# xuekt98/BBDM

Hardware: NVIDIA H100
Metric: denoising-steps/sec (UNet fwd) at 256^2 pixel-BBDM (higher is better)
Workload: dtype bf16x3 (split-bf16 tensor-core products, fp32 accumulate: fp32-class)

## Files before the change

bbdm_b200/cabi.py:

```python
from __future__ import annotations

import ctypes as C
import os

import torch

_HERE = os.path.dirname(os.path.abspath(__file__))
LIB_PATH = os.environ.get("BBDM_LIB") or os.path.join(_HERE, "libbbdm_b200.so")

ABI_VERSION = 3
OBJ = {"grad": 0, "noise": 1, "ysubx": 2}
RESAMPLE_NONE, RESAMPLE_UP2, RESAMPLE_DOWN2 = 0, 1, 2
RES_NONE, RES_SAME, RES_UP2, RES_DOWN2 = 0, 1, 2, 3
GN_MAX_SLICES = 64
ATTN_HEAD_DIMS = (16, 32, 64, 128)
ATTN_TC_HEAD_DIMS = (64, 128)
LN_MAX_C = 2048


def layernorm_bwd_workspace(rows, C):
    return -(-rows // 64) * 2 * C

SYMBOLS = [
    "bbdm_abi_version", "bbdm_last_error", "bbdm_device_info", "bbdm_check_device_fault",
    "bbdm_bridge_q_sample", "bbdm_bridge_p_sample", "bbdm_bridge_p_sample_dev", "bbdm_nchw_to_nhwc_cat", "bbdm_nhwc_to_nchw",
    "bbdm_gather_rows", "bbdm_linear_f32", "bbdm_gn_stats", "bbdm_prep_operand",
    "bbdm_pack_weight_split", "bbdm_pack_weight_split_padded", "bbdm_pack_weight_split_taps", "bbdm_pack_weight_split_dgrad",
    "bbdm_pack_weight_f32", "bbdm_conv_umma", "bbdm_conv_direct",
    "bbdm_attention", "bbdm_attention_split", "bbdm_attention_tc", "bbdm_conv_umma_geometry", "bbdm_gn_finalize_partials",
    "bbdm_split_grad", "bbdm_conv_wgrad_workspace", "bbdm_conv_wgrad", "bbdm_gn_bwd_reduce", "bbdm_gn_bwd_apply",
    "bbdm_conv_wgrad_direct", "bbdm_attention_bwd", "bbdm_conv_direct_pad", "bbdm_softmax_rows_split", "bbdm_vq_nearest", "bbdm_s2d_split", "bbdm_pack_weight_split_both",
    "bbdm_wino_geometry", "bbdm_wino_input", "bbdm_wino_output", "bbdm_wino_pack_weight",
    "bbdm_wino6_geometry", "bbdm_wino6_input", "bbdm_wino6_output", "bbdm_wino6_pack_weight",
# ... 20 lines not shown


class ConvArgs(C.Structure):
    _fields_ = [("B", C.c_int), ("H", C.c_int), ("W", C.c_int),
                ("Cin", C.c_int), ("Cout", C.c_int), ("taps", C.c_int),
                ("a_hi", C.c_void_p), ("a_lo", C.c_void_p), ("w_hi", C.c_void_p), ("w_lo", C.c_void_p),
                ("bias", C.c_void_p),
                ("Cin2", C.c_int),
                ("a2_hi", C.c_void_p), ("a2_lo", C.c_void_p), ("w2_hi", C.c_void_p), ("w2_lo", C.c_void_p),
                ("bias2", C.c_void_p),
                ("residual", C.c_void_p), ("res_mode", C.c_int),
                ("out", C.c_void_p), ("out_hi", C.c_void_p), ("out_lo", C.c_void_p),
                ("passes", C.c_int), ("out_nchw_channels", C.c_int), ("upsample2x", C.c_int),
                ("stats_partial", C.c_void_p), ("weights_per_image", C.c_int), ("operand_f16", C.c_int)]


class WinoInputArgs(C.Structure):
    _fields_ = [("src1", C.c_void_p), ("c1", C.c_int), ("src2", C.c_void_p), ("c2", C.c_int),
                ("B", C.c_int), ("H", C.c_int), ("W", C.c_int), ("groups", C.c_int),
                ("mean", C.c_void_p), ("rstd", C.c_void_p), ("gamma", C.c_void_p), ("beta", C.c_void_p),
                ("film_scale", C.c_void_p), ("film_shift", C.c_void_p), ("film_stride", C.c_int64),
                ("silu", C.c_int),
                ("v_hi", C.c_void_p), ("v_lo", C.c_void_p), ("raw_hi", C.c_void_p), ("raw_lo", C.c_void_p),
                ("act_hi", C.c_void_p), ("act_lo", C.c_void_p)]


class WinoOutputArgs(C.Structure):
    _fields_ = [("m", C.c_void_p), ("inv_wscale", C.c_void_p), ("B", C.c_int), ("H", C.c_int), ("W", C.c_int), ("Cout", C.c_int),
                ("bias", C.c_void_p), ("residual", C.c_void_p), ("res_mode", C.c_int),
                ("out", C.c_void_p), ("stats_partial", C.c_void_p), ("up2_phases", C.c_int)]


class BbdmError(RuntimeError):
    pass


_lib = None


def load():
    global _lib
    if _lib is not None:
        return _lib
    if not os.path.exists(LIB_PATH):
        raise BbdmError(
            f"{LIB_PATH} not found: build the sm_90a kernels first (python -m bbdm_b200.build). "
            "bbdm_b200 has no PyTorch/CPU fallback for its kernels.")
# ... 108 lines not shown
    return cls


LAUNCHES = {"n": 0}


def _req(t, dtype=torch.float32):
    assert t.is_cuda and t.is_contiguous() and t.dtype == dtype, (t.device, t.dtype, t.is_contiguous())
    return t


@_guard_all
class CudaBackend:

    name = "sm_90a"
    requires_cuda = True
    wino_tensor_scale = True
    wino_tiles = (4, 6)

    def __init__(self):
        self.lib = load()

    def empty(self, shape, dtype, device):
        return torch.empty(shape, dtype=dtype, device=device)

    def q_sample(self, x0, y, noise, t, m_t, var_t, objective, xt_out, obj_out):
        B = x0.shape[0]
        n = x0.numel() // B
        for z in (x0, y, noise, m_t, var_t, xt_out, obj_out):
            _req(z)
        _req(t, torch.int64)
        check(self.lib.bbdm_bridge_q_sample(ptr(x0), ptr(y), ptr(noise), ptr(t), ptr(m_t), ptr(var_t),
                                            m_t.numel(), OBJ[objective], ptr(xt_out), ptr(obj_out), B, n,
                                            stream()))
        LAUNCHES["n"] += 1

    def p_sample(self, x_t, y, eps, noise, coef, objective, clip, is_last, x_out, x0_out):
        for z in (x_t, y, eps, x_out):
            _req(z)
        c = PSampleCoef(*[float(v) for v in coef])
        check(self.lib.bbdm_bridge_p_sample(ptr(x_t), ptr(y), ptr(eps), ptr(noise), c, OBJ[objective],
                                            int(clip), int(is_last), ptr(x_out), ptr(x0_out), x_t.numel(),
                                            stream()))
        LAUNCHES["n"] += 1

    def p_sample_dev(self, x_t, y, eps, noise, coef_dev, objective, clip, is_last, x_out, x0_out):
        for z in (x_t, y, eps, x_out, coef_dev):
# ... 78 lines not shown
        a = ConvArgs(B, H, W, Cin, Cout, taps, ptr(a_hi), ptr(a_lo), ptr(w_hi), ptr(w_lo), ptr(bias),
                     Cin2, ptr(a2_hi), ptr(a2_lo), ptr(w2_hi), ptr(w2_lo), ptr(bias2),
                     ptr(residual), res_mode, ptr(out), ptr(out_hi), ptr(out_lo), passes, out_nchw_channels,
                     int(upsample2x), ptr(stats_partial), int(weights_per_image), int(operand_f16))
        check(self.lib.bbdm_conv_umma(C.byref(a), stream()))
        LAUNCHES["n"] += 1

    def conv_geometry(self, H, W):
        v = [C.c_int(0) for _ in range(4)]
        check(self.lib.bbdm_conv_umma_geometry(H, W, *[C.byref(z) for z in v]))
        return tuple(z.value for z in v)

    def _wino(self, name, tile):
        assert tile in self.wino_tiles, tile
        return getattr(self.lib, f"bbdm_wino{'' if tile == 4 else tile}_{name}")

    def wino_geometry(self, B, H, W, tile=4):
        th, tw, el, tot = C.c_int(0), C.c_int(0), C.c_int(0), C.c_int64(0)
        check(self._wino("geometry", tile)(B, H, W, C.byref(th), C.byref(tw), C.byref(tot), C.byref(el)))
        return th.value, tw.value, tot.value, bool(el.value)

    def wino_input(self, src1, src2, *, groups=32, mean=None, rstd=None, gamma=None, beta=None, film_scale=None,
                   film_shift=None, film_stride=0, silu=True, v_hi, v_lo, raw_hi=None, raw_lo=None, act_hi=None,
                   act_lo=None, tile=4):
        B, H, W, c1 = src1.shape
        a = WinoInputArgs(ptr(_req(src1)), c1, ptr(src2), 0 if src2 is None else src2.shape[3], B, H, W, groups,
                          ptr(mean), ptr(rstd), ptr(gamma), ptr(beta), ptr(film_scale), ptr(film_shift), film_stride,
                          int(silu), ptr(_req(v_hi, torch.float16)), ptr(_req(v_lo, torch.float16)),
                          ptr(raw_hi), ptr(raw_lo), ptr(act_hi), ptr(act_lo))
        check(self._wino("input", tile)(C.byref(a), stream()))
        LAUNCHES["n"] += 1

    def wino_output(self, m, *, B, H, W, Cout, bias=None, residual=None, res_mode=RES_NONE, out, stats_partial=None,
                    inv_wscale=None, tile=4, up2_phases=False):
        a = WinoOutputArgs(ptr(_req(m)), None if inv_wscale is None else ptr(_req(inv_wscale)), B, H, W, Cout, ptr(bias), ptr(residual), res_mode, ptr(_req(out)),
                           ptr(stats_partial), int(up2_phases))
        check(self._wino("output", tile)(C.byref(a), stream()))
        LAUNCHES["n"] += 1

    def wino_pack_weight(self, w, u_hi, u_lo, dgrad=False, inv_wscale=None, tile=4):
        Cout, Cin = w.shape[0], w.shape[1]
        check(self._wino("pack_weight", tile)(ptr(_req(w)), Cout, Cin, int(dgrad), ptr(_req(u_hi, torch.float16)),
                                              ptr(_req(u_lo, torch.float16)),
                                              None if inv_wscale is None else ptr(_req(inv_wscale)), stream()))
        LAUNCHES["n"] += 1

    def layernorm_split(self, x, gamma, beta, eps, out_f32=None, out_hi=None, out_lo=None):
        Cc = x.shape[-1]
        check(self.lib.bbdm_layernorm_split(ptr(_req(x)), x.numel() // Cc, Cc, ptr(_req(gamma)), ptr(_req(beta)), eps,
                                            ptr(out_f32), ptr(out_hi), ptr(out_lo), stream()))
        LAUNCHES["n"] += 1

# ... 177 lines not shown
```

bbdm_b200/convs.py:

```python
from __future__ import annotations

import os

import torch

from . import cabi
from .weights import upsample_phase_weights

WINOGRAD = os.environ.get("BBDM_WINOGRAD", "1") != "0"
WINOGRAD_TRAIN = os.environ.get("BBDM_WINOGRAD_TRAIN", "1") != "0"
WINO_MIN_C = int(os.environ.get("BBDM_WINO_MIN_C", "256"))
WINO_MIN_TILES = int(os.environ.get("BBDM_WINO_MIN_TILES", "512"))


def wino_channels_ok(cin, cout, min_c):
    return cin % 64 == 0 and cout % 64 == 0 and min(cin, cout) >= min_c


def wino_tile(H, W):
    f6 = 64 * (-(-H // 6)) * (-(-W // 6))
    f4 = 36 * (H / 4) * (W / 4)
    return 6 if f6 <= 0.9 * f4 else 4


def winograd_ok(geometry, cin, cout, min_c, min_tiles, tile=4):
    th, tw, tiles, ok = geometry
    px = tile * tile
    return bool(ok and wino_channels_ok(cin, cout, min_c) and (th * tw * px >= 128 * 16 or tiles * px >= min_tiles * 16))


class FreshBuffers:

    def __init__(self, device):
        self.device = device

    def get(self, shape, dtype=torch.float32):
        return torch.empty(shape, dtype=dtype, device=self.device)

    def put(self, *ts):
        pass


def wino_conv(be, pool, geometry, src1, src2, *, cout, planes=None, weight=None, dgrad=False, bias=None,
              residual=None, res_mode=cabi.RES_NONE, stats=False, tile=4, up2_phases=False, **transform):
    B, H, W, c1 = src1.shape
    cin = c1 + (0 if src2 is None else src2.shape[3])
    th, _, mtot, _ = geometry
    npos = (tile + 2) ** 2
    tkw = {} if tile == 4 else dict(tile=tile)
    assert not up2_phases or (tile == 6 and planes is not None and residual is None)
    ncols = 4 * cout if up2_phases else cout
    v_hi, v_lo = pool.get((npos, mtot, cin), torch.float16), pool.get((npos, mtot, cin), torch.float16)
    be.wino_input(src1, src2, v_hi=v_hi, v_lo=v_lo, **transform, **tkw)
    if planes is None:
        u_hi, u_lo = pool.get((npos, cout, cin), torch.float16), pool.get((npos, cout, cin), torch.float16)
        u_inv = pool.get((1,)) if getattr(be, "wino_tensor_scale", False) else None
        be.wino_pack_weight(weight.detach().contiguous(), u_hi, u_lo, dgrad=dgrad,
                            **({} if u_inv is None else dict(inv_wscale=u_inv)), **tkw)
    else:
        u_hi, u_lo, u_inv = planes
        assert u_hi.shape[0] == npos, (u_hi.shape, tile)
    m = pool.get((npos, mtot, ncols))
    be.conv_umma(B=npos, H=mtot // 16, W=16, Cin=cin, Cout=ncols, taps=1, a_hi=v_hi, a_lo=v_lo, w_hi=u_hi, w_lo=u_lo,
                 out=m, passes=3, weights_per_image=True, operand_f16=True)
    pool.put(v_hi, v_lo)
    f = 2 if up2_phases else 1
    rows = 4 * th if up2_phases else th
    out = pool.get((B, f * H, f * W, cout))
    part = pool.get((B * rows, cout, 2)) if stats else None
    if up2_phases:
        tkw["up2_phases"] = True
    be.wino_output(m, B=B, H=H, W=W, Cout=cout, bias=bias, residual=residual, res_mode=res_mode, out=out,
                   stats_partial=part, **({} if u_inv is None else dict(inv_wscale=u_inv)), **tkw)
# ... 75 lines not shown
```

bbdm_b200/csrc/winograd.cu:

```cuda
#include "common.cuh"
#include <cuda_fp16.h>
#include <stdlib.h>

namespace bbdm {

constexpr float WINO_WSCALE_FIXED = 256.0f;

__host__ __device__ inline float wino_wscale(uint32_t mbits) {
  if (mbits == 0) return WINO_WSCALE_FIXED;
  const int e = (int)(mbits >> 23) - 127;
  int k = 14 - (e + ((mbits & 0x7fffffu) != 0 ? 1 : 0));
  k = k < -100 ? -100 : (k > 100 ? 100 : k);
  float s = 1.0f;
  for (; k > 0; --k) s *= 2.0f;
  for (; k < 0; ++k) s *= 0.5f;
  return s;
}

template <int S>
__device__ __forceinline__ void wino_bt6(float* d) {
  const float d0 = d[0], d1 = d[S], d2 = d[2 * S], d3 = d[3 * S], d4 = d[4 * S], d5 = d[5 * S];
  d[0] = fmaf(4.0f, d0, fmaf(-5.0f, d2, d4));
  d[S] = fmaf(-4.0f, d1 + d2, d3 + d4);
  d[2 * S] = fmaf(4.0f, d1 - d2, d4 - d3);
// ... 32 lines not shown
  const float a = m[S] + m[2 * S], b = m[S] - m[2 * S];
  const float c = m[3 * S] + m[4 * S], d = m[3 * S] - m[4 * S];
  const float e = m[5 * S] + m[6 * S], f = m[5 * S] - m[6 * S];
  y[0] = ((m[0] + a) + c) + e;
  y[T] = fmaf(2.0f, d, fmaf(0.5f, f, b));
  y[2 * T] = fmaf(4.0f, c, fmaf(0.25f, e, a));
  y[3 * T] = fmaf(8.0f, d, fmaf(0.125f, f, b));
  y[4 * T] = fmaf(16.0f, c, fmaf(0.0625f, e, a));
  y[5 * T] = fmaf(32.0f, d, fmaf(0.03125f, f, b)) + m[7 * S];
}

__device__ __forceinline__ void split2_f16(float a, float b, uint32_t& hi, uint32_t& lo) {
  const __half2 h = __floats2half2_rn(a, b);
  const float2 hf = __half22float2(h);
  const __half2 l = __floats2half2_rn(a - hf.x, b - hf.y);
  hi = *reinterpret_cast<const uint32_t*>(&h);
  lo = *reinterpret_cast<const uint32_t*>(&l);
}

struct WinoInParams {
  const float* src1; int c1;
  const float* src2; int c2;
  int B, H, W, C, groups, cpg, th, tw;
  int64_t Mtot;
  const float* mean; const float* rstd; const float* gamma; const float* beta;
  const float* fscale; const float* fshift; int64_t fstride;
  int silu;
  __half* v_hi; __half* v_lo;
  __nv_bfloat16* raw_hi; __nv_bfloat16* raw_lo;
  __nv_bfloat16* act_hi; __nv_bfloat16* act_lo;
  unsigned long long* fault;
};

constexpr unsigned long long WINO6_RANGE_FAULT = 0xC0000000ull;

template <int VEC>
__global__ void __launch_bounds__(256)
wino_input_kernel(const WinoInParams p) {
  const int b = blockIdx.x / p.th, ty = blockIdx.x % p.th;
  const int c = (blockIdx.y * 256 + threadIdx.x) * VEC;
  if (c >= p.C) return;
  float sc[VEC], sh[VEC];
#pragma unroll
  for (int v = 0; v < VEC; ++v) {
    const int g = (c + v) / p.cpg;
    const float s0 = p.rstd[b * p.groups + g] * p.gamma[c + v];
// ... 89 lines not shown
        const __half h = __float2half_rn(t[0][q]);
        p.v_hi[off] = h;
        p.v_lo[off] = __float2half_rn(t[0][q] - __half2float(h));
      }
    }
  }
}

template <int T>
struct WinoIn {
  static constexpr int N = T + 2;
  static constexpr int CC = 64;
  static constexpr int TX = T == 4 ? 8 : 4;
  static constexpr int COLS = T * TX + 2;
  static constexpr int PATCH = N * COLS * CC;
  static constexpr size_t SMEM = 2 * (size_t)PATCH * sizeof(float);
};
static_assert(WinoIn<4>::SMEM == 2 * 6 * 34 * 64 * 4 && WinoIn<6>::SMEM * 2 <= 227 * 1024, "staged patch budget");

__device__ __forceinline__ void cp_async16(uint32_t saddr, const void* g) {
  asm volatile("cp.async.cg.shared.global [%0], [%1], 16;" ::"r"(saddr), "l"(g) : "memory");
}

template <int T>
__global__ void __launch_bounds__(256, 2)
wino_input_smem_kernel(const WinoInParams p) {
  using K = WinoIn<T>;
  constexpr int N = K::N, CC = K::CC, TX = K::TX, COLS = K::COLS;
  extern __shared__ __align__(16) float patch[];
  const int b = blockIdx.x / p.th, ty = blockIdx.x % p.th;
  const int cbase = blockIdx.y * CC;
  const float* base;
  int cs, cc0;
  if (cbase < p.c1) { base = p.src1; cs = p.c1; cc0 = cbase; } else { base = p.src2; cs = p.c2; cc0 = cbase - p.c1; }
  const int y0 = T * ty - 1;
  const int tid = threadIdx.x;
  const int ch4 = tid & 15;
  const int pix0 = tid >> 4;
  constexpr int NPIX = N * COLS;

  if constexpr (T == 6) {
    if (blockIdx.x == 0) {
      const int64_t tiles = (int64_t)p.B * p.th * p.tw;
      const int npad = (int)(p.Mtot - tiles);
      for (int k = tid; k < N * N * npad * CC; k += 256) {
        const int c = k % CC, r = (k / CC) % npad, q = k / (CC * npad);
        const int64_t off = ((int64_t)q * p.Mtot + tiles + r) * p.C + cbase + c;
        p.v_hi[off] = __float2half_rn(0.f);
        p.v_lo[off] = __float2half_rn(0.f);
      }
    }
  }

  float sc[4], sh[4];
#pragma unroll
  for (int v = 0; v < 4; ++v) {
    sc[v] = 1.0f; sh[v] = 0.0f;
    if (p.mean) {
      const int c = cbase + ch4 * 4 + v;
      const int g = c / p.cpg;
      const float s0 = p.rstd[b * p.groups + g] * p.gamma[c];
      const float h0 = p.beta[c] - p.mean[b * p.groups + g] * s0;
      float f1 = 1.0f, f0 = 0.0f;
      if (p.fscale) { f1 = 1.0f + p.fscale[(int64_t)b * p.fstride + c]; f0 = p.fshift[(int64_t)b * p.fstride + c]; }
      sc[v] = s0 * f1;
      sh[v] = fmaf(h0, f1, f0);
    }
  }
  const int nseg = (p.tw + TX - 1) / TX;
  const uint32_t patch_s = (uint32_t)__cvta_generic_to_shared(patch);

  auto stage = [&](int seg, int buf) {
    const int x0 = T * TX * seg - 1;
    int i = 0, j = pix0;
    for (int px = pix0; px < NPIX; px += 16, j += 16) {
      if (j >= COLS) { j -= COLS; ++i; }
      const int iy = y0 + i, ix = x0 + j;
      if (iy >= 0 && iy < p.H && ix >= 0 && ix < p.W)
        cp_async16(patch_s + (uint32_t)(((buf * NPIX + px) * CC + ch4 * 4) * 4),
                   base + (((int64_t)b * p.H + iy) * p.W + ix) * cs + cc0 + ch4 * 4);
    }
    asm volatile("cp.async.commit_group;" ::: "memory");
  };

  stage(0, 0);
  for (int seg = 0; seg < nseg; ++seg) {
    const int buf = seg & 1;
    if (seg + 1 < nseg) {
      stage(seg + 1, buf ^ 1);
      asm volatile("cp.async.wait_group 1;" ::: "memory");
    } else {
      asm volatile("cp.async.wait_group 0;" ::: "memory");
    }
    __syncthreads();
    float* pb = patch + buf * K::PATCH;
    const int x0 = T * TX * seg - 1;
    int i = 0, j = pix0;
    for (int px = pix0; px < NPIX; px += 16, j += 16) {
      if (j >= COLS) { j -= COLS; ++i; }
      const int iy = y0 + i, ix = x0 + j;
      float4* q = reinterpret_cast<float4*>(pb + px * CC + ch4 * 4);
      float4 a = make_float4(0.f, 0.f, 0.f, 0.f);
      if (iy >= 0 && iy < p.H && ix >= 0 && ix < p.W) {
        const float4 x = *q;
        if (p.raw_hi && i >= 1 && i <= T && j >= 1 && j <= T * TX) {
          uint2 h, l;
          split4(x, h, l);
          const int64_t off = (((int64_t)b * p.H + iy) * p.W + ix) * p.C + cbase + ch4 * 4;
          *reinterpret_cast<uint2*>(p.raw_hi + off) = h;
          *reinterpret_cast<uint2*>(p.raw_lo + off) = l;
        }
        a.x = fmaf(x.x, sc[0], sh[0]); a.y = fmaf(x.y, sc[1], sh[1]);
        a.z = fmaf(x.z, sc[2], sh[2]); a.w = fmaf(x.w, sc[3], sh[3]);
        if (p.silu) {
          a.x = __fdividef(a.x, 1.0f + __expf(-a.x)); a.y = __fdividef(a.y, 1.0f + __expf(-a.y));
          a.z = __fdividef(a.z, 1.0f + __expf(-a.z)); a.w = __fdividef(a.w, 1.0f + __expf(-a.w));
        }
        if (p.act_hi && i >= 1 && i <= T && j >= 1 && j <= T * TX) {
          uint2 h, l;
          split4(a, h, l);
          const int64_t off = (((int64_t)b * p.H + iy) * p.W + ix) * p.C + cbase + ch4 * 4;
          *reinterpret_cast<uint2*>(p.act_hi + off) = h;
          *reinterpret_cast<uint2*>(p.act_lo + off) = l;
        }
      }
      *q = a;
    }
    __syncthreads();
    const int64_t plane = p.Mtot * p.C;
    if constexpr (T == 4) {
      const int txl = tid >> 5, c0 = (tid & 31) * 2;
      const int tx = TX * seg + txl;
      if (tx < p.tw) {
        float t0[36], t1[36];
#pragma unroll
        for (int i = 0; i < 6; ++i)
#pragma unroll
          for (int j = 0; j < 6; ++j) {
            const float2 v = *reinterpret_cast<const float2*>(pb + ((i * COLS + 4 * txl + j) * CC + c0));
            t0[i * 6 + j] = v.x;
// ... 315 lines not shown
        u_lo[off] = l;
      }
    }
  }
}

}

using namespace bbdm;

namespace {

template <int T>
int wino_geometry_t(int B, int H, int W, int* tiles_h, int* tiles_w, int64_t* tiles_total, int* eligible) {
  BBDM_REQUIRE(B > 0 && H > 0 && W > 0, "wino_geometry: bad shape");
  const int th = T == 4 ? H / 4 : (H + 5) / 6, tw = T == 4 ? W / 4 : (W + 5) / 6;
  int64_t mtot = (int64_t)B * th * tw;
  if (T == 6) mtot = mtot < 128 ? 128 : (mtot + 15) / 16 * 16;
  if (tiles_h) *tiles_h = th;
  if (tiles_w) *tiles_w = tw;
  if (tiles_total) *tiles_total = mtot;
  const bool aligned = T == 6 || (H % 4 == 0 && W % 4 == 0);
  if (eligible) *eligible = (aligned && mtot % 16 == 0 && mtot >= 128) ? 1 : 0;
  return BBDM_OK;
}

template <int T>
int wino_input_t(const BbdmWinoInputArgs* a, void* stream) {
  BBDM_REQUIRE(a && a->src1 && a->v_hi && a->v_lo, "wino_input: null args");
  WinoInParams p;
  p.src1 = a->src1; p.c1 = a->c1;
  p.src2 = a->src2; p.c2 = a->src2 ? a->c2 : 0;
  p.B = a->B; p.H = a->H; p.W = a->W;
  p.C = p.c1 + p.c2;
  p.groups = a->groups;
  if (T == 4)
    BBDM_REQUIRE(p.B > 0 && p.H > 0 && p.W > 0 && p.H % 4 == 0 && p.W % 4 == 0, "wino_input: H, W must be multiples of 4");
  else
    BBDM_REQUIRE(p.B > 0 && p.H > 0 && p.W > 0, "wino6_input: bad shape");
  BBDM_REQUIRE(p.c1 % 2 == 0 && p.c2 % 2 == 0 && p.C > 0, "wino_input: channel counts must be even");
  if (a->mean) {
    BBDM_REQUIRE(a->rstd && a->gamma && a->beta && p.groups > 0 && p.C % p.groups == 0, "wino_input: incomplete GroupNorm args");
  } else {
    BBDM_REQUIRE(!a->silu && !a->film_scale, "wino_input: identity mode (mean == NULL) takes no activation / FiLM");
    if (p.groups <= 0) p.groups = 1;
  }
  BBDM_REQUIRE((a->act_hi == nullptr) == (a->act_lo == nullptr), "wino_input: act hi/lo must come in pairs");
  BBDM_REQUIRE((a->film_scale == nullptr) == (a->film_shift == nullptr), "wino_input: film scale/shift mismatch");
  BBDM_REQUIRE((a->raw_hi == nullptr) == (a->raw_lo == nullptr), "wino_input: raw hi/lo must come in pairs");
  p.cpg = p.C / p.groups;
  wino_geometry_t<T>(p.B, p.H, p.W, &p.th, &p.tw, &p.Mtot, nullptr);
  p.mean = a->mean; p.rstd = a->rstd; p.gamma = a->gamma; p.beta = a->beta;
  p.fscale = a->film_scale; p.fshift = a->film_shift; p.fstride = a->film_stride;
  p.silu = a->silu;
  p.v_hi = (__half*)a->v_hi; p.v_lo = (__half*)a->v_lo;
  p.raw_hi = (__nv_bfloat16*)a->raw_hi; p.raw_lo = (__nv_bfloat16*)a->raw_lo;
  p.act_hi = (__nv_bfloat16*)a->act_hi; p.act_lo = (__nv_bfloat16*)a->act_lo;
  p.fault = nullptr;
  if (T == 6) {
    p.fault = device_fault_ptr();
    BBDM_REQUIRE(p.fault != nullptr, "wino6_input: device fault word unavailable");
  }
  const bool smem_only = a->mean == nullptr || a->act_hi != nullptr;
  const int64_t ctas = (int64_t)p.B * p.th;
  BBDM_REQUIRE(ctas < (1ll << 31), "wino_input: too many tile rows");
  constexpr int CC = WinoIn<T>::CC;
  static int vec = -1;
  if (vec < 0) { const char* e = getenv("BBDM_WINO_IN_VEC"); vec = e ? (atoi(e) == 2 ? 2 : 1) : 0; }
  if ((T == 6 || vec == 0) && p.c1 % CC == 0 && p.c2 % CC == 0) {
    static DeviceOnce configured;
    if (configured.need()) {
      BBDM_CUDA_CHECK(cudaFuncSetAttribute(wino_input_smem_kernel<T>, cudaFuncAttributeMaxDynamicSharedMemorySize,
                                           (int)WinoIn<T>::SMEM));
      configured.mark();
    }
    dim3 grid((unsigned)ctas, p.C / CC);
    wino_input_smem_kernel<T><<<grid, 256, WinoIn<T>::SMEM, (cudaStream_t)stream>>>(p);
  } else if (T == 6) {
    BBDM_REQUIRE(false, "wino6_input: channel counts must be multiples of 64");
  } else if (smem_only) {
    BBDM_REQUIRE(false, "wino_input: identity mode / act planes need channel counts that are multiples of 64");
  } else if (vec == 2 || (vec == 0 && p.c1 % 2 == 0 && p.c2 % 2 == 0)) {
    dim3 grid((unsigned)ctas, (p.C / 2 + 255) / 256);
    wino_input_kernel<2><<<grid, 256, 0, (cudaStream_t)stream>>>(p);
  } else {
    dim3 grid((unsigned)ctas, (p.C + 255) / 256);
    wino_input_kernel<1><<<grid, 256, 0, (cudaStream_t)stream>>>(p);
  }
  BBDM_LAUNCH_CHECK();
  return BBDM_OK;
}

template <int T>
int wino_output_t(const BbdmWinoOutputArgs* a, void* stream) {
  BBDM_REQUIRE(a && a->m && a->out, "wino_output: null args");
  WinoOutParams p;
  p.m = a->m; p.inv_wscale = a->inv_wscale;
  p.B = a->B; p.H = a->H; p.W = a->W; p.Cout = a->Cout;
  if (T == 4)
    BBDM_REQUIRE(p.B > 0 && p.B <= 65535 && p.H > 0 && p.W > 0 && p.H % 4 == 0 && p.W % 4 == 0,
// ... 82 lines not shown
```

bbdm_b200/engine.py:

```python
from __future__ import annotations

import torch
import torch.nn as nn

from . import cabi, convs
from .transformer import SpatialTransformer
from .unet import (AttentionBlock, Downsample, ResBlock, TimestepEmbedSequential, UNetModel,
                   Upsample, timestep_embedding)

GN_GROUPS = 32
GN_EPS = 1e-5


def resample_to_res(resample):
    return {cabi.RESAMPLE_NONE: cabi.RES_SAME, cabi.RESAMPLE_UP2: cabi.RES_UP2,
            cabi.RESAMPLE_DOWN2: cabi.RES_DOWN2}[resample]


class _Pool:

    _serial = 0

    def __init__(self, backend, device):
        self.be, self.device, self.free = backend, device, {}
# ... 193 lines not shown
        fuse_skip = es is not None and umma2 and es["k"] == 1 and cin % 64 == 0
        need_raw_f32 = (es is not None and not fuse_skip) or \
                       (es is None and (src2 is not None or (resample != cabi.RESAMPLE_NONE and not umma2)))
        r_f32 = r_hi = r_lo = None

        mean, rstd = self._stats(pool, src1, src2)
        gkw = dict(groups=GN_GROUPS, mean=mean, rstd=rstd, gamma=norm1.weight.detach(), beta=norm1.bias.detach(),
                   silu=True)
        up_phase = resample == cabi.RESAMPLE_UP2 and umma1 and "up_hi" in e1 and Ws >= 4 and bias1 is None \
            and not need_raw_f32 and not fuse_skip
        if up_phase and self.wino and "up6" in e1 and c1 % 64 == 0:
            u = e1["up6"]
            h1 = convs.wino_conv(be, pool, self._wino_geometry(B, Hs, Ws, 6), src1, src2, cout=cout,
                                 planes=(u["u_hi"], u["u_lo"], u.get("u_inv")), bias=e1["bias"], stats=True, tile=6,
                                 up2_phases=True, **gkw)
            pool.put(mean, rstd)
        elif up_phase:
            a_hi, a_lo = pool.get((B, Hs, Ws, cin), torch.bfloat16), pool.get((B, Hs, Ws, cin), torch.bfloat16)
            be.prep(src1, src2, **gkw, resample=cabi.RESAMPLE_NONE, act_hi=a_hi, act_lo=a_lo)
            pool.put(mean, rstd)
            h1, _, _ = self._conv(pool, e1, a_hi=a_hi, a_lo=a_lo, shape=(B, Hs, Ws), planes=(e1["up_hi"], e1["up_lo"]),
                                  taps=4, upsample2x=True, stats=True)
            pool.put(a_hi, a_lo)
        elif umma1 and resample == cabi.RESAMPLE_NONE and not need_raw_f32 and bias1 is None \
                and self._wino_ok(e1, B, H, W, c1):
            if fuse_skip:
                r_hi, r_lo = pool.get(shp, torch.bfloat16), pool.get(shp, torch.bfloat16)
            h1 = self._wino_conv(pool, e1, src1, src2, **gkw, raw_hi=r_hi, raw_lo=r_lo)
            pool.put(mean, rstd)
        else:
            a_f32 = a_hi = a_lo = None
            if umma1:
                a_hi, a_lo = pool.get(shp, torch.bfloat16), pool.get(shp, torch.bfloat16)
            else:
                a_f32 = pool.get(shp)
            if fuse_skip:
                r_hi, r_lo = pool.get(shp, torch.bfloat16), pool.get(shp, torch.bfloat16)
            if need_raw_f32:
                r_f32 = pool.get(shp)
            be.prep(src1, src2, **gkw, resample=resample, act_f32=a_f32, act_hi=a_hi, act_lo=a_lo,
                    raw_f32=r_f32, raw_hi=r_hi, raw_lo=r_lo)
            pool.put(mean, rstd)
            if bias1 is None:
                h1, _, _ = self._conv(pool, e1, a_f32=a_f32, a_hi=a_hi, a_lo=a_lo, shape=shape, stats=True)
            else:
                h1 = pool.get((B, H, W, cout))
                for b in range(B):
                    sl = lambda z: None if z is None else z[b:b + 1]
                    self._conv(pool, e1, a_f32=sl(a_f32), a_hi=sl(a_hi), a_lo=sl(a_lo), shape=(1, H, W),
                               bias=bias1[b], out=h1[b:b + 1])
            pool.put(a_f32, a_hi, a_lo)
# ... 32 lines not shown
        key = (H, W)
        r = self._geom_cache.get(key)
        if r is None:
            r = self._geom_cache[key] = self.be.conv_geometry(H, W)[3]
        return r


    def _wino_geometry(self, B, H, W, tile=4):
        key = (B, H, W, tile)
        g = self._wino_geom.get(key)
        if g is None:
            g = self._wino_geom[key] = self.be.wino_geometry(B, H, W, **({} if tile == 4 else dict(tile=tile)))
        return g

    def _wino_ok(self, ent, B, H, W, c1=None):
        if not (self.wino and "u_hi" in ent):
            return False
        tile = ent["u_tile"]
        if tile == 6 and c1 is not None and c1 % 64:
            return False
        return convs.winograd_ok(self._wino_geometry(B, H, W, tile), ent["cin"], ent["cout"], self.wino_min_c,
                                 self.wino_min_tiles, tile)

    def _wino_ready(self, ent):
        return self.wino and "hi" in ent and ent["k"] == 3 and convs.wino_channels_ok(ent["cin"], ent["cout"],
                                                                                     self.wino_min_c)

    def _wino_conv(self, pool, ent, src1, src2, *, residual=None, res_mode=cabi.RES_NONE, **transform):
        B, H, W, _ = src1.shape
        tile = ent["u_tile"]
        return convs.wino_conv(self.be, pool, self._wino_geometry(B, H, W, tile), src1, src2, cout=ent["cout"],
                               planes=(ent["u_hi"], ent["u_lo"], ent.get("u_inv")), bias=ent["bias"],
                               residual=residual, res_mode=res_mode, stats=True, tile=tile, **transform)


class UNetEngine(KernelExecutor):
    def __init__(self, unet: UNetModel, backend=None, precision: str = "split3"):
        super().__init__(backend, precision)
        self.unet = unet
        self._wkey = None
        self._w = {}
        self._table = None
        self.num_timesteps = 1000
        self.generation = 0

    def _params_key(self):
        return tuple((p.data_ptr(), p._version) for p in self.unet.parameters())

    @staticmethod
    def _ptrs(key):
        return None if key is None else tuple(k[0] for k in key)

    def refresh_weights(self, force=False):
        key = self._params_key()
        if not force and key == self._wkey:
            return
# ... 17 lines not shown
                if not m.use_scale_shift_norm:
                    b = b + m.in_layers[2].bias.detach()
                film_w.append(lin.weight.detach())
                film_b.append(b)
                w[name + "#film"] = (off, n)
                off += n
        for name, m in u.named_modules():
            if isinstance(m, SpatialTransformer):
                for j, blk in enumerate(m.transformer_blocks):
                    pre = f"{name}.transformer_blocks.{j}"
                    a1, a2 = blk.attn1, blk.attn2
                    packer.conv(pre + ".attn1.qkv", torch.cat([a1.to_q.weight, a1.to_k.weight, a1.to_v.weight], 0), None)
                    packer.conv(pre + ".attn1.to_out.0", a1.to_out[0].weight, a1.to_out[0].bias)
                    packer.conv(pre + ".attn2.to_q", a2.to_q.weight, None)
                    packer.conv(pre + ".attn2.to_kv", torch.cat([a2.to_k.weight, a2.to_v.weight], 0), None)
                    packer.conv(pre + ".attn2.to_out.0", a2.to_out[0].weight, a2.to_out[0].bias)
                    packer.conv(pre + ".ff.net.0.proj", blk.ff.net[0].proj.weight, blk.ff.net[0].proj.bias)
                    packer.conv(pre + ".ff.net.2", blk.ff.net[2].weight, blk.ff.net[2].bias)
        sizes = self._resblock_sizes()
        for name, m in u.named_modules():
            if isinstance(m, ResBlock) and m.use_scale_shift_norm:
                hw = sizes[name]
                tile = convs.wino_tile(hw, hw) if 6 in getattr(be, "wino_tiles", (4,)) else 4
                for cname, conv, resampled in ((name + ".in_layers.2", m.in_layers[2], m.up or m.down),
                                               (name + ".out_layers.3", m.out_layers[3], False)):
                    if not resampled and self._wino_ready(w[cname]):
                        packer.winograd(cname, conv.weight, tile)
        for name, m in u.named_modules():
            if isinstance(m, ResBlock) and m.up and m.channels % 64 == 0 and m.out_channels % 64 == 0:
                packer.up_phase(name + ".in_layers.2", m.in_layers[2].weight)
                low = sizes[name] // 2
                if self.wino and 6 in getattr(be, "wino_tiles", (4,)) and convs.wino_tile(low, low) == 6:
                    packer.up_phase_winograd(name + ".in_layers.2", m.in_layers[2].weight)
        if old and old.get("film_n") == off and old["film_w"].device == dev:
            w["film_w"], w["film_b"] = old["film_w"], old["film_b"]
            torch.cat(film_w, 0, out=w["film_w"])
            torch.cat(film_b, 0, out=w["film_b"])
        else:
            w["film_w"] = torch.cat(film_w, 0).contiguous()
            w["film_b"] = torch.cat(film_b, 0).contiguous()
        w["film_n"] = off
        self._w = w
        self._wkey = key

    def _resblock_sizes(self):
        u, side, out = self.unet, int(self.unet.image_size), {}
        for prefix, blocks in (("input_blocks", u.input_blocks), ("middle_block", [u.middle_block]),
                               ("output_blocks", u.output_blocks)):
            for i, block in enumerate(blocks):
# ... 226 lines not shown
```

include/bbdm_b200.h:

```cpp
#ifndef BBDM_B200_H_
#define BBDM_B200_H_

#include <stdint.h>

#ifdef __cplusplus
extern "C" {
#endif

#define BBDM_ABI_VERSION 3

enum {
  BBDM_OK = 0,
  BBDM_E_INVALID = -1,
  BBDM_E_CUDA = -2,
  BBDM_E_UNSUPPORTED = -3,
  BBDM_E_DEVICE = -4
};

int bbdm_abi_version(void);
const char* bbdm_last_error(void);
int bbdm_device_info(int* sm_count, int* cc_major, int* cc_minor);
int bbdm_check_device_fault(void* stream, unsigned long long* fault_word);


enum { BBDM_OBJ_GRAD = 0, BBDM_OBJ_NOISE = 1, BBDM_OBJ_YSUBX = 2 };

int bbdm_bridge_q_sample(const float* x0, const float* y, const float* noise, const int64_t* t,
                         const float* m_t, const float* variance_t, int num_timesteps,
                         int objective, float* x_t_out, float* objective_out,
                         int B, int64_t n_per_sample, void* stream);

typedef struct {
// ... 87 lines not shown
} BbdmConvArgs;
int bbdm_conv_umma(const BbdmConvArgs* a, void* stream);

int bbdm_conv_umma_geometry(int H, int W, int* TW, int* TH, int* TB, int* rows_per_image);

int bbdm_gn_finalize_partials(const float* part1, int c1, int rows1, const float* part2, int c2,
                              int rows2, int B, int hw, int groups, float eps, float* mean,
                              float* rstd, void* stream);


int bbdm_wino_geometry(int B, int H, int W, int* tiles_h, int* tiles_w, int64_t* tiles_total, int* eligible);

typedef struct {
  const float* src1; int c1;
  const float* src2; int c2;
  int B, H, W;
  int groups;
  const float* mean; const float* rstd; const float* gamma; const float* beta;
  const float* film_scale; const float* film_shift; int64_t film_stride;
  int silu;
  void* v_hi; void* v_lo;
  void* raw_hi; void* raw_lo;
  void* act_hi; void* act_lo;
} BbdmWinoInputArgs;
int bbdm_wino_input(const BbdmWinoInputArgs* a, void* stream);

typedef struct {
  const float* m;
  const float* inv_wscale;
  int B, H, W, Cout;
  const float* bias;
  const float* residual; int res_mode;
  float* out;
  float* stats_partial;
  int up2_phases;
} BbdmWinoOutputArgs;
int bbdm_wino_output(const BbdmWinoOutputArgs* a, void* stream);

int bbdm_wino_pack_weight(const float* w, int Cout, int Cin, int dgrad, void* u_hi, void* u_lo, float* inv_wscale,
                          void* stream);

int bbdm_wino6_geometry(int B, int H, int W, int* tiles_h, int* tiles_w, int64_t* tiles_total, int* eligible);
int bbdm_wino6_input(const BbdmWinoInputArgs* a, void* stream);
int bbdm_wino6_output(const BbdmWinoOutputArgs* a, void* stream);
int bbdm_wino6_pack_weight(const float* w, int Cout, int Cin, int dgrad, void* u_hi, void* u_lo, float* inv_wscale,
                           void* stream);
// ... 93 lines not shown
```

Baseline: 5.830.

## Fuse 2x avg-pool downsample into F(6,3) Winograd input transform for down ResBlocks

Adds a pooled variant of the F(6,3) Winograd input kernel. It reads four source pixels, applies GroupNorm/FiLM/SiLU to each, and averages them, so downsampling ResBlocks' first conv can run through Winograd instead of the direct/UMMA path. It also widens the channel-eligibility rule for tile-6 convs with cin>=256, cout>=128, so more layers get Winograd weights packed. The pooled path loads directly from global memory rather than through cp.async staging, which may lower input-stage bandwidth. An OOM retry with gc.collect is added to buffer allocation.

```diff
diff --git a/bbdm_b200/cabi.py b/bbdm_b200/cabi.py
--- a/bbdm_b200/cabi.py
+++ b/bbdm_b200/cabi.py
@@ -1,6 +1,7 @@
 from __future__ import annotations
 
 import ctypes as C
+import gc
 import os
 
 import torch
@@ -8,7 +9,7 @@
 _HERE = os.path.dirname(os.path.abspath(__file__))
 LIB_PATH = os.environ.get("BBDM_LIB") or os.path.join(_HERE, "libbbdm_b200.so")
 
-ABI_VERSION = 3
+ABI_VERSION = 4
 OBJ = {"grad": 0, "noise": 1, "ysubx": 2}
 RESAMPLE_NONE, RESAMPLE_UP2, RESAMPLE_DOWN2 = 0, 1, 2
 RES_NONE, RES_SAME, RES_UP2, RES_DOWN2 = 0, 1, 2, 3
@@ -75,7 +76,7 @@
                 ("film_scale", C.c_void_p), ("film_shift", C.c_void_p), ("film_stride", C.c_int64),
                 ("silu", C.c_int),
                 ("v_hi", C.c_void_p), ("v_lo", C.c_void_p), ("raw_hi", C.c_void_p), ("raw_lo", C.c_void_p),
-                ("act_hi", C.c_void_p), ("act_lo", C.c_void_p)]
+                ("act_hi", C.c_void_p), ("act_lo", C.c_void_p), ("down2", C.c_int)]
 
 
 class WinoOutputArgs(C.Structure):
@@ -230,7 +231,11 @@
         self.lib = load()
 
     def empty(self, shape, dtype, device):
-        return torch.empty(shape, dtype=dtype, device=device)
+        try:
+            return torch.empty(shape, dtype=dtype, device=device)
+        except torch.OutOfMemoryError:
+            gc.collect()
+            return torch.empty(shape, dtype=dtype, device=device)
 
     def q_sample(self, x0, y, noise, t, m_t, var_t, objective, xt_out, obj_out):
         B = x0.shape[0]
@@ -355,12 +360,12 @@
 
     def wino_input(self, src1, src2, *, groups=32, mean=None, rstd=None, gamma=None, beta=None, film_scale=None,
                    film_shift=None, film_stride=0, silu=True, v_hi, v_lo, raw_hi=None, raw_lo=None, act_hi=None,
-                   act_lo=None, tile=4):
+                   act_lo=None, tile=4, down2=False):
         B, H, W, c1 = src1.shape
         a = WinoInputArgs(ptr(_req(src1)), c1, ptr(src2), 0 if src2 is None else src2.shape[3], B, H, W, groups,
                           ptr(mean), ptr(rstd), ptr(gamma), ptr(beta), ptr(film_scale), ptr(film_shift), film_stride,
                           int(silu), ptr(_req(v_hi, torch.float16)), ptr(_req(v_lo, torch.float16)),
-                          ptr(raw_hi), ptr(raw_lo), ptr(act_hi), ptr(act_lo))
+                          ptr(raw_hi), ptr(raw_lo), ptr(act_hi), ptr(act_lo), int(down2))
         check(self._wino("input", tile)(C.byref(a), stream()))
         LAUNCHES["n"] += 1
 
diff --git a/bbdm_b200/convs.py b/bbdm_b200/convs.py
--- a/bbdm_b200/convs.py
+++ b/bbdm_b200/convs.py
@@ -13,8 +13,12 @@
 WINO_MIN_TILES = int(os.environ.get("BBDM_WINO_MIN_TILES", "512"))
 
 
-def wino_channels_ok(cin, cout, min_c):
-    return cin % 64 == 0 and cout % 64 == 0 and min(cin, cout) >= min_c
+def wino_channels_ok(cin, cout, min_c, tile=4):
+    if cin % 64 or cout % 64:
+        return False
+    if min(cin, cout) >= min_c:
+        return True
+    return tile == 6 and cin >= 256 and cout >= 128
 
 
 def wino_tile(H, W):
@@ -26,7 +30,8 @@
 def winograd_ok(geometry, cin, cout, min_c, min_tiles, tile=4):
     th, tw, tiles, ok = geometry
     px = tile * tile
-    return bool(ok and wino_channels_ok(cin, cout, min_c) and (th * tw * px >= 128 * 16 or tiles * px >= min_tiles * 16))
+    return bool(ok and wino_channels_ok(cin, cout, min_c, tile) and
+                (th * tw * px >= 128 * 16 or tiles * px >= min_tiles * 16))
 
 
 class FreshBuffers:
@@ -42,13 +47,17 @@
 
 
 def wino_conv(be, pool, geometry, src1, src2, *, cout, planes=None, weight=None, dgrad=False, bias=None,
-              residual=None, res_mode=cabi.RES_NONE, stats=False, tile=4, up2_phases=False, **transform):
+              residual=None, res_mode=cabi.RES_NONE, stats=False, tile=4, up2_phases=False, down2=False, **transform):
     B, H, W, c1 = src1.shape
     cin = c1 + (0 if src2 is None else src2.shape[3])
     th, _, mtot, _ = geometry
     npos = (tile + 2) ** 2
     tkw = {} if tile == 4 else dict(tile=tile)
     assert not up2_phases or (tile == 6 and planes is not None and residual is None)
+    assert not down2 or (tile == 6 and not up2_phases)
+    if down2:
+        H, W = H // 2, W // 2
+        transform["down2"] = True
     ncols = 4 * cout if up2_phases else cout
     v_hi, v_lo = pool.get((npos, mtot, cin), torch.float16), pool.get((npos, mtot, cin), torch.float16)
     be.wino_input(src1, src2, v_hi=v_hi, v_lo=v_lo, **transform, **tkw)
diff --git a/bbdm_b200/csrc/winograd.cu b/bbdm_b200/csrc/winograd.cu
--- a/bbdm_b200/csrc/winograd.cu
+++ b/bbdm_b200/csrc/winograd.cu
@@ -78,6 +78,7 @@
   const float* src1; int c1;
   const float* src2; int c2;
   int B, H, W, C, groups, cpg, th, tw;
+  int sH, sW;
   int64_t Mtot;
   const float* mean; const float* rstd; const float* gamma; const float* beta;
   const float* fscale; const float* fshift; int64_t fstride;
@@ -213,9 +214,10 @@
   asm volatile("cp.async.cg.shared.global [%0], [%1], 16;" ::"r"(saddr), "l"(g) : "memory");
 }
 
-template <int T>
+template <int T, bool POOL>
 __global__ void __launch_bounds__(256, 2)
 wino_input_smem_kernel(const WinoInParams p) {
+  static_assert(!POOL || T == 6, "the pooled input form is F(6,3) only");
   using K = WinoIn<T>;
   constexpr int N = K::N, CC = K::CC, TX = K::TX, COLS = K::COLS;
   extern __shared__ __align__(16) float patch[];
@@ -262,16 +264,27 @@
   const uint32_t patch_s = (uint32_t)__cvta_generic_to_shared(patch);
 
   auto stage = [&](int seg, int buf) {
-    const int x0 = T * TX * seg - 1;
-    int i = 0, j = pix0;
-    for (int px = pix0; px < NPIX; px += 16, j += 16) {
-      if (j >= COLS) { j -= COLS; ++i; }
-      const int iy = y0 + i, ix = x0 + j;
-      if (iy >= 0 && iy < p.H && ix >= 0 && ix < p.W)
-        cp_async16(patch_s + (uint32_t)(((buf * NPIX + px) * CC + ch4 * 4) * 4),
-                   base + (((int64_t)b * p.H + iy) * p.W + ix) * cs + cc0 + ch4 * 4);
+    if constexpr (!POOL) {
+      const int x0 = T * TX * seg - 1;
+      int i = 0, j = pix0;
+      for (int px = pix0; px < NPIX; px += 16, j += 16) {
+        if (j >= COLS) { j -= COLS; ++i; }
+        const int iy = y0 + i, ix = x0 + j;
+        if (iy >= 0 && iy < p.H && ix >= 0 && ix < p.W)
+          cp_async16(patch_s + (uint32_t)(((buf * NPIX + px) * CC + ch4 * 4) * 4),
+                     base + (((int64_t)b * p.H + iy) * p.W + ix) * cs + cc0 + ch4 * 4);
+      }
     }
     asm volatile("cp.async.commit_group;" ::: "memory");
+  };
+  auto activate = [&](const float4 x) {
+    float4 a = make_float4(fmaf(x.x, sc[0], sh[0]), fmaf(x.y, sc[1], sh[1]), fmaf(x.z, sc[2], sh[2]),
+                           fmaf(x.w, sc[3], sh[3]));
+    if (p.silu) {
+      a.x = __fdividef(a.x, 1.0f + __expf(-a.x)); a.y = __fdividef(a.y, 1.0f + __expf(-a.y));
+      a.z = __fdividef(a.z, 1.0f + __expf(-a.z)); a.w = __fdividef(a.w, 1.0f + __expf(-a.w));
+    }
+    return a;
   };
 
   stage(0, 0);
@@ -292,7 +305,16 @@
       const int iy = y0 + i, ix = x0 + j;
       float4* q = reinterpret_cast<float4*>(pb + px * CC + ch4 * 4);
       float4 a = make_float4(0.f, 0.f, 0.f, 0.f);
-      if (iy >= 0 && iy < p.H && ix >= 0 && ix < p.W) {
+      if (POOL && iy >= 0 && iy < p.H && ix >= 0 && ix < p.W) {
+        const float* s = base + (((int64_t)b * p.sH + 2 * iy) * p.sW + 2 * ix) * cs + cc0 + ch4 * 4;
+        const int64_t rs = (int64_t)p.sW * cs;
+        const float4 a0 = activate(__ldg(reinterpret_cast<const float4*>(s)));
+        const float4 a1 = activate(__ldg(reinterpret_cast<const float4*>(s + cs)));
+        const float4 a2 = activate(__ldg(reinterpret_cast<const float4*>(s + rs)));
+        const float4 a3 = activate(__ldg(reinterpret_cast<const float4*>(s + rs + cs)));
+        a = make_float4(0.25f * (((a0.x + a1.x) + a2.x) + a3.x), 0.25f * (((a0.y + a1.y) + a2.y) + a3.y),
+                        0.25f * (((a0.z + a1.z) + a2.z) + a3.z), 0.25f * (((a0.w + a1.w) + a2.w) + a3.w));
+      } else if (!POOL && iy >= 0 && iy < p.H && ix >= 0 && ix < p.W) {
         const float4 x = *q;
         if (p.raw_hi && i >= 1 && i <= T && j >= 1 && j <= T * TX) {
           uint2 h, l;
@@ -301,12 +323,7 @@
           *reinterpret_cast<uint2*>(p.raw_hi + off) = h;
           *reinterpret_cast<uint2*>(p.raw_lo + off) = l;
         }
-        a.x = fmaf(x.x, sc[0], sh[0]); a.y = fmaf(x.y, sc[1], sh[1]);
-        a.z = fmaf(x.z, sc[2], sh[2]); a.w = fmaf(x.w, sc[3], sh[3]);
-        if (p.silu) {
-          a.x = __fdividef(a.x, 1.0f + __expf(-a.x)); a.y = __fdividef(a.y, 1.0f + __expf(-a.y));
-          a.z = __fdividef(a.z, 1.0f + __expf(-a.z)); a.w = __fdividef(a.w, 1.0f + __expf(-a.w));
-        }
+        a = activate(x);
         if (p.act_hi && i >= 1 && i <= T && j >= 1 && j <= T * TX) {
           uint2 h, l;
           split4(a, h, l);
@@ -668,6 +685,19 @@
   if (tiles_total) *tiles_total = mtot;
   const bool aligned = T == 6 || (H % 4 == 0 && W % 4 == 0);
   if (eligible) *eligible = (aligned && mtot % 16 == 0 && mtot >= 128) ? 1 : 0;
+  return BBDM_OK;
+}
+
+template <int T, bool POOL>
+int launch_wino_input_smem(const WinoInParams& p, dim3 grid, void* stream) {
+  static DeviceOnce configured;
+  if (configured.need()) {
+    BBDM_CUDA_CHECK(cudaFuncSetAttribute(wino_input_smem_kernel<T, POOL>, cudaFuncAttributeMaxDynamicSharedMemorySize,
+                                         (int)WinoIn<T>::SMEM));
+    configured.mark();
+  }
+  wino_input_smem_kernel<T, POOL><<<grid, 256, WinoIn<T>::SMEM, (cudaStream_t)stream>>>(p);
+  BBDM_LAUNCH_CHECK();
   return BBDM_OK;
 }
 
@@ -695,6 +725,12 @@
   BBDM_REQUIRE((a->film_scale == nullptr) == (a->film_shift == nullptr), "wino_input: film scale/shift mismatch");
   BBDM_REQUIRE((a->raw_hi == nullptr) == (a->raw_lo == nullptr), "wino_input: raw hi/lo must come in pairs");
   p.cpg = p.C / p.groups;
+  p.sH = p.H; p.sW = p.W;
+  if (a->down2) {
+    BBDM_REQUIRE(T == 6 && !a->raw_hi && !a->act_hi && p.H >= 2 && p.W >= 2,
+                 "wino_input: down2 is an F(6,3) form without raw / act planes (H, W >= 2)");
+    p.H /= 2; p.W /= 2;
+  }
   wino_geometry_t<T>(p.B, p.H, p.W, &p.th, &p.tw, &p.Mtot, nullptr);
   p.mean = a->mean; p.rstd = a->rstd; p.gamma = a->gamma; p.beta = a->beta;
   p.fscale = a->film_scale; p.fshift = a->film_shift; p.fstride = a->film_stride;
@@ -714,14 +750,11 @@
   static int vec = -1;
   if (vec < 0) { const char* e = getenv("BBDM_WINO_IN_VEC"); vec = e ? (atoi(e) == 2 ? 2 : 1) : 0; }
   if ((T == 6 || vec == 0) && p.c1 % CC == 0 && p.c2 % CC == 0) {
-    static DeviceOnce configured;
-    if (configured.need()) {
-      BBDM_CUDA_CHECK(cudaFuncSetAttribute(wino_input_smem_kernel<T>, cudaFuncAttributeMaxDynamicSharedMemorySize,
-                                           (int)WinoIn<T>::SMEM));
-      configured.mark();
-    }
-    dim3 grid((unsigned)ctas, p.C / CC);
-    wino_input_smem_kernel<T><<<grid, 256, WinoIn<T>::SMEM, (cudaStream_t)stream>>>(p);
+    const dim3 grid((unsigned)ctas, p.C / CC);
+    if constexpr (T == 6) {
+      if (a->down2) return launch_wino_input_smem<T, true>(p, grid, stream);
+    }
+    return launch_wino_input_smem<T, false>(p, grid, stream);
   } else if (T == 6) {
     BBDM_REQUIRE(false, "wino6_input: channel counts must be multiples of 64");
   } else if (smem_only) {
diff --git a/bbdm_b200/engine.py b/bbdm_b200/engine.py
--- a/bbdm_b200/engine.py
+++ b/bbdm_b200/engine.py
@@ -239,11 +239,13 @@
             h1, _, _ = self._conv(pool, e1, a_hi=a_hi, a_lo=a_lo, shape=(B, Hs, Ws), planes=(e1["up_hi"], e1["up_lo"]),
                                   taps=4, upsample2x=True, stats=True)
             pool.put(a_hi, a_lo)
-        elif umma1 and resample == cabi.RESAMPLE_NONE and not need_raw_f32 and bias1 is None \
-                and self._wino_ok(e1, B, H, W, c1):
+        elif umma1 and not need_raw_f32 and bias1 is None and (
+                resample == cabi.RESAMPLE_NONE or (resample == cabi.RESAMPLE_DOWN2 and e1.get("u_tile") == 6
+                                                   and not fuse_skip)) and self._wino_ok(e1, B, H, W, c1):
             if fuse_skip:
                 r_hi, r_lo = pool.get(shp, torch.bfloat16), pool.get(shp, torch.bfloat16)
-            h1 = self._wino_conv(pool, e1, src1, src2, **gkw, raw_hi=r_hi, raw_lo=r_lo)
+            h1 = self._wino_conv(pool, e1, src1, src2, **gkw, raw_hi=r_hi, raw_lo=r_lo,
+                                 down2=resample == cabi.RESAMPLE_DOWN2)
             pool.put(mean, rstd)
         else:
             a_f32 = a_hi = a_lo = None
@@ -322,16 +324,17 @@
         return convs.winograd_ok(self._wino_geometry(B, H, W, tile), ent["cin"], ent["cout"], self.wino_min_c,
                                  self.wino_min_tiles, tile)
 
-    def _wino_ready(self, ent):
+    def _wino_ready(self, ent, tile=4):
         return self.wino and "hi" in ent and ent["k"] == 3 and convs.wino_channels_ok(ent["cin"], ent["cout"],
-                                                                                     self.wino_min_c)
-
-    def _wino_conv(self, pool, ent, src1, src2, *, residual=None, res_mode=cabi.RES_NONE, **transform):
+                                                                                     self.wino_min_c, tile)
+
+    def _wino_conv(self, pool, ent, src1, src2, *, residual=None, res_mode=cabi.RES_NONE, down2=False, **transform):
         B, H, W, _ = src1.shape
+        f = 2 if down2 else 1
         tile = ent["u_tile"]
-        return convs.wino_conv(self.be, pool, self._wino_geometry(B, H, W, tile), src1, src2, cout=ent["cout"],
-                               planes=(ent["u_hi"], ent["u_lo"], ent.get("u_inv")), bias=ent["bias"],
-                               residual=residual, res_mode=res_mode, stats=True, tile=tile, **transform)
+        return convs.wino_conv(self.be, pool, self._wino_geometry(B, H // f, W // f, tile), src1, src2,
+                               cout=ent["cout"], planes=(ent["u_hi"], ent["u_lo"], ent.get("u_inv")), bias=ent["bias"],
+                               residual=residual, res_mode=res_mode, stats=True, tile=tile, down2=down2, **transform)
 
 
 class UNetEngine(KernelExecutor):
@@ -395,9 +398,9 @@
             if isinstance(m, ResBlock) and m.use_scale_shift_norm:
                 hw = sizes[name]
                 tile = convs.wino_tile(hw, hw) if 6 in getattr(be, "wino_tiles", (4,)) else 4
-                for cname, conv, resampled in ((name + ".in_layers.2", m.in_layers[2], m.up or m.down),
-                                               (name + ".out_layers.3", m.out_layers[3], False)):
-                    if not resampled and self._wino_ready(w[cname]):
+                for cname, conv, direct in ((name + ".in_layers.2", m.in_layers[2], m.up or (m.down and tile != 6)),
+                                            (name + ".out_layers.3", m.out_layers[3], False)):
+                    if not direct and self._wino_ready(w[cname], tile):
                         packer.winograd(cname, conv.weight, tile)
         for name, m in u.named_modules():
             if isinstance(m, ResBlock) and m.up and m.channels % 64 == 0 and m.out_channels % 64 == 0:
diff --git a/include/bbdm_b200.h b/include/bbdm_b200.h
--- a/include/bbdm_b200.h
+++ b/include/bbdm_b200.h
@@ -7,7 +7,7 @@
 extern "C" {
 #endif
 
-#define BBDM_ABI_VERSION 3
+#define BBDM_ABI_VERSION 4
 
 enum {
   BBDM_OK = 0,
@@ -141,6 +141,7 @@
   void* v_hi; void* v_lo;
   void* raw_hi; void* raw_lo;
   void* act_hi; void* act_lo;
+  int down2;
 } BbdmWinoInputArgs;
 int bbdm_wino_input(const BbdmWinoInputArgs* a, void* stream);
 
```

Measured after the change: 6.084, median of 6. 1.04x the previous value.
